# at-aaims/OmniFed

Hardware: AMD Instinct MI355X
Metric: GB/s device-resident QSGD encode+decode, Llama-400M grads, 1/2/4/8 GPUs (higher is better)
Workload: dtype f32; 1 GPU; llama400m QSGD encode+decode, bit_width 4 (16 levels, int8 wire), philox draws, client weighting fused (alpha = batch_samples = rank + 1), one client per GPU; tensors=183, elements_per_client=401122304, bit_width=4, parallelism=clients1

## Files before the change

omnifed_amd/csrc/omf_plan.h:

```cpp
#pragma once

#include <algorithm>
#include <vector>

#include "../../include/omf_codec.h"
#include "omf_common.h"
#include "omf_plan_layout.h"

namespace omf {

constexpr uint64_t kWaitTicks = 2000000ull;

struct SpecBracket {
  float c_lo, c_hi, n_lo, n_hi;
  uint32_t mode;
  uint32_t pad[3];
};

}

struct omf_plan {
  int device = 0;
  int32_t nt = 0;
  int64_t chunk = omf::plan_layout::kSub;
// ... 9 lines not shown
  void* d_block = nullptr;
  uint8_t* d_sync = nullptr;
  size_t sync_bytes = 0, off_counters = 16, off_gran = 0;
  int64_t n_enc[2] = {0, 0};
  omf::plan_layout::Item* d_enc[2] = {nullptr, nullptr};
  int64_t n_flat = 0, n_partials = 0;
  omf::plan_layout::Item* d_flat = nullptr;
  omf::plan_layout::TensorInfo* d_tinfo[2] = {nullptr, nullptr};
  uint64_t* d_partials = nullptr;
  int64_t* d_sizes = nullptr;
  int64_t* d_begins = nullptr;
  int32_t ring_cfg = 0;
  int32_t ring_grid = 0;
  int32_t ring_big_mode = 1;
  int64_t ring_gap = -1;
  int64_t ring_hold_override = 0;
  uint32_t ring_dbg = 0;
  uint32_t ring_epoch = 0;
  int64_t n_ring = 0, n_ring_gran = 0, ring_hold_max = 0, ring_two_pass = 0;
  omf::ring::Item* d_ring = nullptr;
  omf::ring::Tensor* d_ring_t = nullptr;
  uint64_t* d_ring_gran = nullptr;
  unsigned long long* d_ring_prof = nullptr;
  int64_t n_spec_blocks = 0, n_spec_fold = 0;
  omf::plan_layout::SpecBrItem* d_spec_br_items = nullptr;
  omf::plan_layout::SpecFoldItem* d_spec_fold_items = nullptr;
  uint64_t* d_spec_seg_part = nullptr;
  uint32_t* d_spec_cnt = nullptr;
  omf::SpecBracket* d_spec_br = nullptr;
  uint64_t* d_spec_ngran = nullptr;
  uint64_t* d_spec_part = nullptr;
  uint32_t* d_spec_slots = nullptr;
  uint32_t* d_spec_heads = nullptr;
  int64_t n_dec_blocks = 0;
  uint32_t* d_dec_binfo = nullptr;
  float4* d_spec_recs = nullptr;
  uint32_t* d_spec_flags = nullptr;
  uint32_t* d_spec_status = nullptr;
  int32_t grid_wgs = 0;
  uint32_t* d_grid_pbeg = nullptr;
  uint32_t* d_grid_pcnt = nullptr;
  unsigned long long* d_grid_bar = nullptr;
  uint64_t grid_launches = 0;
  uint32_t spec_epoch = 0;
  uint32_t spec_skip = 0;
  float spec_zsig = 5.0f;
  float spec_zsig_wide = 4.0f;
  int32_t spec_fb = 1;
  int32_t spec_wide = 1;
  int32_t spec_last_pw = 0;
  std::vector<void*> d_lazy;
  uint32_t* d_spec_slots_w = nullptr;
  float4* d_spec_recs_w = nullptr;
  double* d_spec_br_part = nullptr;
  uint32_t* d_spec_br_cnt = nullptr;
  double* d_spec_fb_part = nullptr;
  uint32_t* d_spec_fb_cnt = nullptr;
  uint64_t* d_spec_brgran = nullptr;
  struct TopkTable {
    uint64_t key;
    void* dev;
    uint64_t host;
    std::vector<int64_t> counts;
  };
  std::vector<TopkTable> topk_tables;
  omf::TopkKnobs topk_knobs;
// ... 69 lines not shown
```

omnifed_amd/csrc/omf_plan_layout.cpp:

```cpp
#include "omf_plan_layout.h"

#include <algorithm>
#include <utility>

namespace omf {
namespace plan_layout {

namespace {

void build_sequence(const Desc& d, bool resident_ok, std::vector<Item>& seq, std::vector<TensorInfo>& tinfo,
                    int64_t& npart) {
  seq.clear();
  tinfo.assign(d.nt, TensorInfo{});
  npart = 0;
  std::vector<Item> deferred;
  for (int32_t t = 0; t < d.nt; ++t) {
    const int64_t n = d.sizes[t], b = d.offsets[t];
    const int64_t es = (int64_t)d.ev * 1024;
    const int64_t ns = (n + es - 1) / es;
    std::vector<Item> q_t;
    if (ns == 1 || (resident_ok && ns <= d.cap)) {
      tinfo[t] = TensorInfo{b, n, es, (int32_t)ns, (int32_t)npart};
      for (int64_t c = 0; c < ns; ++c) {
        const int64_t cb = b + c * es;
// ... 151 lines not shown
    const int64_t p_begin = kItemParts * (int64_t)o.flat.size();
    for (int64_t c = 0; c * kSub < n; ++c) {
      const int64_t cb = b + c * kSub;
      o.flat.push_back(Item{cb, std::min(b + n, cb + kSub), t, kQuant, (int32_t)c, 0});
    }
    const int64_t p_end = kItemParts * (int64_t)o.flat.size();
    o.grid_pbeg[(size_t)t] = (uint32_t)(p_begin / kItemParts);
    o.grid_pcnt[(size_t)t] = (uint32_t)((p_end - p_begin) / kItemParts);
    const int64_t R = std::max<int64_t>(1, std::min<int64_t>(kSpecRuns, n / (2 * kSpecRun)));
    const int64_t Rw = std::max<int64_t>(1, std::min<int64_t>(kSpecRunsWide, n / (2 * kSpecRunWide)));
    o.br_items.push_back(SpecBrItem{b, n, n / R, (int32_t)R, (int32_t)(n % R), t, (int32_t)Rw});
    const int32_t nsegs = (int32_t)((p_end - p_begin + kSpecSeg - 1) / kSpecSeg);
    for (int32_t q = 0; q < nsegs; ++q)
      o.fold_items.push_back(SpecFoldItem{p_begin + (int64_t)q * kSpecSeg,
                                          std::min(p_end, p_begin + (int64_t)(q + 1) * kSpecSeg), t, q, nsegs, seg_base});
    seg_base += nsegs;
  }
}

void build_dec_blocks(const Desc& d, std::vector<uint32_t>& binfo) {
  const int64_t arena_end = d.offsets[d.nt - 1] + d.sizes[d.nt - 1];
  binfo.assign((size_t)((arena_end + kDecBlk - 1) / kDecBlk), 0u);
  int32_t t = 0;
  for (size_t k = 0; k < binfo.size(); ++k) {
    const int64_t base = (int64_t)k * kDecBlk;
    while (t + 1 < d.nt && d.offsets[t + 1] <= base) ++t;
    const bool inside = d.offsets[t] <= base && base + kDecBlk <= d.offsets[t] + d.sizes[t];
    binfo[k] = (uint32_t)t | (inside ? 0x80000000u : 0u);
  }
}

}

bool build_tables(const Desc& d, Tables& o) {
  int64_t np[2];
  build_sequence(d, true, o.enc[0], o.tinfo[0], np[0]);
  build_sequence(d, false, o.enc[1], o.tinfo[1], np[1]);
  build_ring_sequence(d, o);
  build_flat_tables(d, o);
  build_dec_blocks(d, o.dec_binfo);
  o.n_enc[0] = (int64_t)o.enc[0].size();
  o.n_enc[1] = (int64_t)o.enc[1].size();
  o.n_flat = (int64_t)o.flat.size();
  o.n_spec_blocks = 4 * o.n_flat;
  o.n_partials = std::max<int64_t>(std::max(np[0], np[1]), 1);
  return std::max(o.n_enc[0], o.n_spec_blocks) <= 0x7fffffffLL;
}

Choice choose_encoder(const Call& c) {
  const bool int32_wire = c.bits > 6;
  const int32_t ordered = c.strategy >= 2 ? kEncOrdered : c.strategy;
  if (c.norms_only) return {(Encoder)ordered};
  if (c.caller_norms) return {kEncCallerNorms};
  if (c.strategy == 4 && !c.caller_u && !c.divide && c.grid_fits) return {kEncGrid};
  if (c.strategy == 3 && !c.caller_u && c.bits >= kSpecMinBits) {
    const bool wide = c.bits > kSpecMaxBits;
    const bool serves = wide ? !c.last_client && c.wide_levels && c.bits <= kSpecMaxBitsWide && c.fmt == 0
                             : c.fmt == 0 || !c.divide;
    if (serves) {
      const bool skip_bracket = (c.spec_dbg & 1u) != 0;
      const bool fused = c.fused_bracket && !c.last_client && c.fmt == 0 && !skip_bracket;
      return {kEncBracket, wide, fused, !fused && !skip_bracket};
    }
  }
  const bool wide_ring = c.strategy == 3 && int32_wire && !c.caller_u && c.fmt == 0;
  if (c.strategy == 2 || c.strategy == 4 || c.divide || wide_ring) return {kEncRing};
  return {(Encoder)ordered};
}

}
}
```

omnifed_amd/csrc/omf_plan_layout.h:

```cpp
#pragma once

#include <cstddef>
#include <cstdint>
#include <vector>

namespace omf {

namespace ring {

enum : int32_t { kPublish = 1, kQuant = 2 };

struct Item {
  int64_t begin, end;
  int64_t tbegin, tn;
  int32_t tensor, flags, chunk, nchunks;
  int32_t gbase, pad[3];
};

struct Tensor {
  int64_t begin, n;
  int32_t nchunks, gbase;
  int32_t pad[2];
};

}

namespace plan_layout {

constexpr int kBlkWaves = 4;
constexpr int64_t kSub = 16384;
constexpr int64_t kSpecBlk = 4096;
constexpr int64_t kDecBlk = 4096;
constexpr int kSpecSeg = 4096;
constexpr int kSpecRun = 64;
constexpr int kSpecRuns = 512;
constexpr int kSpecRunWide = 256;
constexpr int kSpecRunsWide = 512;
#ifndef OMF_BR_PARTS
#define OMF_BR_PARTS 2
#endif
constexpr int kBrParts = OMF_BR_PARTS;
constexpr int kFbParts = 8;
#ifndef OMF_WFB_PARTS
#define OMF_WFB_PARTS 16
#endif
constexpr int kWfbParts = OMF_WFB_PARTS;
constexpr int kGridNB = 3;
constexpr int kSpecMinBits = 1;
constexpr int kSpecMaxBits = 4;
constexpr int kSpecMaxBitsWide = 8;
static_assert(kSub == 4 * kSpecBlk, "four spec blocks per flat item");

enum : int32_t { kNorm = 0, kQuant = 1, kResident = 2 };

struct Item {
  int64_t begin, end;
  int32_t tensor, kind, chunk, pad;
};

struct TensorInfo {
  int64_t begin, n;
  int64_t chunk;
  int32_t nchunks, pbase;
};

struct SpecBrItem {
  int64_t begin, n;
  int64_t base;
  int32_t R, rem;
  int32_t tensor, Rw;
};
struct SpecFoldItem {
  int64_t p_begin, p_end;
  int32_t tensor, seg, nsegs, sbase;
};

struct Desc {
  const int64_t* sizes = nullptr;
  const int64_t* offsets = nullptr;
  int32_t nt = 0;
  int64_t chunk = 2 * kSub;
  int32_t ev = 8;
  int64_t cap = 1;
  int64_t ring_chunk = kSub;
  int32_t ring_slots = 1, ring_kind = 0;
  int32_t ring_grid = 1;
  int32_t ring_big_mode = 1;
  int64_t ring_gap = -1;
  int64_t ring_hold_override = 0;
};

struct Tables {
  std::vector<Item> enc[2];
  std::vector<TensorInfo> tinfo[2];
  std::vector<Item> flat;
  std::vector<ring::Item> ring;
  std::vector<ring::Tensor> ring_t;
  std::vector<SpecBrItem> br_items;
  std::vector<SpecFoldItem> fold_items;
  std::vector<uint32_t> grid_pbeg, grid_pcnt;
  std::vector<uint32_t> dec_binfo;
  int64_t n_enc[2] = {0, 0}, n_flat = 0;
  int64_t n_partials = 0;
  int64_t n_spec_blocks = 0;
  int64_t n_ring_gran = 0;
  int64_t ring_hold_max = 0;
  int64_t ring_two_pass = 0;
};

bool build_tables(const Desc& d, Tables& out);

inline size_t round16(size_t b) { return (b + 15) & ~(size_t)15; }

class Carve {
 public:
  struct Region {
    size_t offset, bytes;
    const void* src;
    bool zero;
    void* field;
    void (*set)(void* field, void* addr);
  };
  template <class T>
  void copy(T*& field, const std::vector<T>& host) { add(field, host.size(), host.data(), false); }
  template <class T>
  void copy(T*& field, const T* host, size_t count) { add(field, count, host, false); }
  template <class T>
  void zero(T*& field, size_t count) { add(field, count, static_cast<const T*>(nullptr), true); }
  template <class T>
  void raw(T*& field, size_t count) { add(field, count, static_cast<const T*>(nullptr), false); }
  size_t bytes() const { return total_; }
  const std::vector<Region>& regions() const { return regions_; }
  void bind(void* base) const {
// ... 48 lines not shown
```

omnifed_amd/csrc/omf_qsgd.hip:

```cpp
#include <algorithm>
#include <cstdlib>
#include <cstring>
#include <type_traits>
#include <vector>

#include "../../include/omf_codec.h"
#include "../../include/omf_codec_experimental.h"
#include "omf_common.h"
#include "omf_plan.h"
#include "omf_qsgd_dev.h"
#include "omf_ring.h"

using namespace omf;
using namespace omf::plan_layout;

namespace {

constexpr int kV = 16;
static_assert(kSub == (int64_t)kV * kThreads * 4, "a flat item is one sub-chunk of a 256-thread workgroup");
static_assert(kBlkWaves == kWaves, "one wave partial per wave of a block's workgroup");

struct EncArgs {
  const float* x;
  const float* u;
// ... 796 lines not shown
        }
      }
      float acc = 0.0f;
#pragma unroll
      for (int i = 0; i < 4; ++i) acc = sq4(spec_prologue(v[i], a.e.alpha, a.divisor, a.e.fmt), acc);
      s1 += (double)acc;
    }
  } else {
    bracket_sample<kSpecRun, false, kThreads, 4>(a, x, t, tb, n, R, part, kFbParts, s1, s2);
  }
  double S1 = block_sum_f64(s1, red), S2 = block_sum_f64(s2, red);
  if (!exact) {
    if (threadIdx.x == 0) {
      double* bp = a.br_part + 2 * ((int64_t)t * kFbParts + part);
      st_agent(reinterpret_cast<uint64_t*>(bp), (uint64_t)__double_as_longlong(S1));
      st_agent(reinterpret_cast<uint64_t*>(bp + 1), (uint64_t)__double_as_longlong(S2));
      drain_vmem();
      const uint32_t last = add_agent(&a.br_cnt[t], 1u) == (uint32_t)(kFbParts - 1) ? 1u : 0u;
      if (last) __hip_atomic_store(&a.br_cnt[t], 0u, __ATOMIC_RELAXED, __HIP_MEMORY_SCOPE_AGENT);
      s_last = last;
    }
    __syncthreads();
    if (!s_last) return;
    S1 = S2 = 0.0;
    for (int g = 0; g < kFbParts; ++g) {
      const uint64_t* bp = reinterpret_cast<const uint64_t*>(a.br_part + 2 * ((int64_t)t * kFbParts + g));
      S1 += __longlong_as_double((long long)ld_agent(bp));
      S2 += __longlong_as_double((long long)ld_agent(bp + 1));
    }
  }
  if (threadIdx.x != 0) return;
  const SpecBracket o = bracket_from_sums(a, exact, n, R, kSpecRun, S1, S2);
  a.br[t] = o;
  const uint64_t ep = (uint64_t)a.epoch << 32;
  st_agent(&a.brgran[2 * t], ep | __float_as_uint(o.c_lo));
  st_agent(&a.brgran[2 * t + 1], ep | __float_as_uint(o.c_hi));
}

template <int WIDTH, bool DIV>
__global__ __launch_bounds__(kThreads) void qsgd_spec_quant_fb(SpecArgs a, const SpecBrItem* __restrict__ bitems,
                                                               int64_t nbrw, const int64_t* __restrict__ begins) {
  if ((int64_t)blockIdx.x < nbrw) {
    spec_bracket_part(a, bitems, blockIdx.x);
    return;
  }
  const int64_t blk = (int64_t)blockIdx.x - nbrw;
  const Item it = a.e.items[blk >> 2];
  const int32_t t = it.tensor;
  const int64_t tb = begins[t];
  const int64_t b = it.begin + (blk & 3) * kSpecBlk;
  const int wave = threadIdx.x >> 6;
  uint32_t* slot = a.slots + blk * kSpecSlot;
  uint64_t* part = a.partials + blk * kWaves + wave;
  if (b >= it.end) {
    if ((threadIdx.x & 63) == 0) {
      *part = 0ull;
      a.heads[blk * kWaves + wave] = (uint32_t)t << 8;
    }
    return;
  }
  auto get_br = [&]() {
    uint64_t g0 = ld_agent(&a.brgran[2 * t]), g1 = ld_agent(&a.brgran[2 * t + 1]);
    if ((uint32_t)(g0 >> 32) != a.epoch || (uint32_t)(g1 >> 32) != a.epoch) {
      const uint64_t t0 = wall_clock64(), min_polls = a.wait_ticks >> 10;
      uint64_t polls = 0;
      for (int k = 0;; k = min(k + 1, 6)) {
        if (k < 2) __builtin_amdgcn_s_sleep(2);
        else __builtin_amdgcn_s_sleep(8);
        g0 = ld_agent(&a.brgran[2 * t]);
        g1 = ld_agent(&a.brgran[2 * t + 1]);
        if ((uint32_t)(g0 >> 32) == a.epoch && (uint32_t)(g1 >> 32) == a.epoch) break;
        if (++polls > min_polls && wall_clock64() - t0 > a.wait_ticks) {
          __hip_atomic_fetch_or(&a.flags[t], 2u, __ATOMIC_RELAXED, __HIP_MEMORY_SCOPE_AGENT);
          g0 = g1 = 0;
          break;
        }
      }
    }
    SpecBracket o{__uint_as_float((uint32_t)g0), __uint_as_float((uint32_t)g1), 0.f, 0.f, 0u, {0u, 0u, 0u}};
    return o;
// ... 28 lines not shown
        v[i] = e + 4 <= n ? *reinterpret_cast<const float4*>(x + e) : make_float4(0.f, 0.f, 0.f, 0.f);
        if (e < n && e + 4 > n) {
          v[i].x = x[e];
          if (e + 1 < n) v[i].y = x[e + 1];
          if (e + 2 < n) v[i].z = x[e + 2];
        }
      }
      float acc = 0.0f;
#pragma unroll
      for (int i = 0; i < 4; ++i) acc = sq4(spec_prologue(v[i], a.e.alpha, a.divisor, a.e.fmt), acc);
      s1 += (double)acc;
    }
  } else {
    bracket_sample<kSpecRunWide, false, 64, kPassesW>(a, x, t, tb, n, R, part, kWfbParts, s1, s2);
  }
  double S1 = wave_sum_f64(s1), S2 = wave_sum_f64(s2);
  if (lane != 0) return;
  if (!exact) {
    double* bp = a.br_part + 2 * ((int64_t)t * kWfbParts + part);
    st_agent(reinterpret_cast<uint64_t*>(bp), (uint64_t)__double_as_longlong(S1));
    st_agent(reinterpret_cast<uint64_t*>(bp + 1), (uint64_t)__double_as_longlong(S2));
    drain_vmem();
    if (add_agent(&a.br_cnt[t], 1u) != (uint32_t)(kWfbParts - 1)) return;
    __hip_atomic_store(&a.br_cnt[t], 0u, __ATOMIC_RELAXED, __HIP_MEMORY_SCOPE_AGENT);
    S1 = S2 = 0.0;
    for (int g = 0; g < kWfbParts; ++g) {
      const uint64_t* q = reinterpret_cast<const uint64_t*>(a.br_part + 2 * ((int64_t)t * kWfbParts + g));
      S1 += __longlong_as_double((long long)ld_agent(q));
      S2 += __longlong_as_double((long long)ld_agent(q + 1));
    }
  }
  const SpecBracket o = bracket_from_sums(a, exact, n, R, kSpecRunWide, S1, S2);
  a.br[t] = o;
  const uint64_t ep = (uint64_t)a.epoch << 32;
  st_agent(&a.brgran[2 * t], ep | __float_as_uint(o.c_lo));
  st_agent(&a.brgran[2 * t + 1], ep | __float_as_uint(o.c_hi));
}

__device__ __forceinline__ SpecBracket fb_poll(const SpecArgs& a, int32_t t) {
  uint64_t g0 = ld_agent(&a.brgran[2 * t]), g1 = ld_agent(&a.brgran[2 * t + 1]);
  if ((uint32_t)(g0 >> 32) != a.epoch || (uint32_t)(g1 >> 32) != a.epoch) {
    const uint64_t t0 = wall_clock64(), min_polls = a.wait_ticks >> 10;
    uint64_t polls = 0;
    for (int k = 0;; k = min(k + 1, 6)) {
      if (k < 2) __builtin_amdgcn_s_sleep(2);
      else __builtin_amdgcn_s_sleep(8);
      g0 = ld_agent(&a.brgran[2 * t]);
      g1 = ld_agent(&a.brgran[2 * t + 1]);
      if ((uint32_t)(g0 >> 32) == a.epoch && (uint32_t)(g1 >> 32) == a.epoch) break;
      if (++polls > min_polls && wall_clock64() - t0 > a.wait_ticks) {
        __hip_atomic_fetch_or(&a.flags[t], 2u, __ATOMIC_RELAXED, __HIP_MEMORY_SCOPE_AGENT);
        g0 = g1 = 0;
        break;
      }
    }
  }
  return SpecBracket{__uint_as_float((uint32_t)g0), __uint_as_float((uint32_t)g1), 0.f, 0.f, 0u, {0u, 0u, 0u}};
}

template <int WIDTH, bool DIV>
__global__ __launch_bounds__(64) void qsgd_spec_quant_wfb(SpecArgs a, const SpecBrItem* __restrict__ bitems,
                                                          int64_t nbrw, const int64_t* __restrict__ begins) {
  if ((int64_t)blockIdx.x < nbrw) {
    spec_bracket_part_wide(a, bitems, blockIdx.x);
    return;
  }
  const int64_t wgi = (int64_t)blockIdx.x - nbrw;
  const int64_t blk = wgi / kWaves;
  const int tid = (int)(wgi % kWaves) * 64 + (int)threadIdx.x;
  const Item it = a.e.items[blk >> 2];
  const int32_t t = it.tensor;
  const int64_t tb = begins[t];
  const int64_t b = it.begin + (blk & 3) * kSpecBlk;
  const int wave = tid >> 6;
  uint32_t* slot = a.slots + blk * spec_slot_words(kSpecPerWaveWide);
  uint64_t* part = a.partials + blk * kWaves + wave;
  if (b >= it.end) {
    if (threadIdx.x == 0) {
      *part = 0ull;
      a.heads[blk * kWaves + wave] = (uint32_t)t << 8;
    }
    return;
  }
  auto get_br = [&]() { return fb_poll(a, t); };
  const int64_t end = min(b + kSpecBlk, it.end);
  if (end - b == kSpecBlk)
    spec_block<WIDTH, true, DIV, kFmtF32, 0, kSpecPerWaveWide>(a, blk, b, end, t, tb, get_br, slot, part, 0.0f, tid);
  else
    spec_block<WIDTH, false, DIV, kFmtF32, 0, kSpecPerWaveWide>(a, blk, b, end, t, tb, get_br, slot, part, 0.0f, tid);
}

__device__ void spec_fold(const SpecArgs& a, const SpecFoldItem& fi) {
  __shared__ double red[kWaves];
  __shared__ uint32_t s_last;
  const int32_t t = fi.tensor;
  constexpr int U = kSpecSeg / kThreads;
  double v[U];
#pragma unroll
  for (int i = 0; i < U; ++i) {
    const int64_t j = fi.p_begin + threadIdx.x + (int64_t)i * kThreads;
    const double d = __longlong_as_double((long long)a.partials[j < fi.p_end ? j : fi.p_begin]);
    v[i] = j < fi.p_end ? d : 0.0;
  }
// ... 651 lines not shown
    for (const Carve::Region& r : c.regions()) {
      void* dst = static_cast<uint8_t*>(*block) + r.offset;
      if (!r.bytes) continue;
      if (r.src) OMF_HIP(hipMemcpy(dst, r.src, r.bytes, hipMemcpyHostToDevice));
      else if (r.zero) OMF_HIP(hipMemset(dst, 0, r.bytes));
    }
    return OMF_OK;
  };
  const int rc = fill();
  if (rc != OMF_OK && *block) {
    (void)hipFree(*block);
    *block = nullptr;
  }
  c.bind(*block);
  return rc;
}

static int upload_plan(omf_plan* p) {
  const ring::Config rc = ring::config(p->ring_cfg);
  Desc d;
  d.sizes = p->sizes.data();
  d.offsets = p->offsets.data();
  d.nt = p->nt;
  d.chunk = p->chunk;
  d.ev = p->ev;
  d.cap = p->cap;
  d.ring_chunk = ring::chunk_elems(rc);
  d.ring_slots = rc.slots;
  d.ring_kind = rc.kind;
  d.ring_grid = p->ring_grid;
  d.ring_big_mode = p->ring_big_mode;
  d.ring_gap = p->ring_gap;
  d.ring_hold_override = p->ring_hold_override;
  Tables tb;
  if (!build_tables(d, tb)) return fail(OMF_EINVAL, "too many work items");
  p->n_enc[0] = tb.n_enc[0];
  p->n_enc[1] = tb.n_enc[1];
  p->n_flat = tb.n_flat;
  p->n_partials = tb.n_partials;
  p->n_ring = (int64_t)tb.ring.size();
  p->n_ring_gran = tb.n_ring_gran;
  p->ring_hold_max = tb.ring_hold_max;
  p->ring_two_pass = tb.ring_two_pass;
  p->n_spec_blocks = tb.n_spec_blocks;
  p->n_spec_fold = (int64_t)tb.fold_items.size();
  p->n_dec_blocks = (int64_t)tb.dec_binfo.size();
  p->off_counters = 16;
  p->off_gran = round16(p->off_counters + 4 * (size_t)p->nt);
  p->sync_bytes = round16(p->off_gran + 8 * (size_t)p->nt);
  const size_t nt = (size_t)p->nt, nb = (size_t)p->n_spec_blocks;
  Carve c;
  c.zero(p->d_sync, p->sync_bytes);
  c.copy(p->d_enc[0], tb.enc[0]);
  c.copy(p->d_enc[1], tb.enc[1]);
  c.copy(p->d_flat, tb.flat);
  c.copy(p->d_tinfo[0], tb.tinfo[0]);
  c.copy(p->d_tinfo[1], tb.tinfo[1]);
  c.raw(p->d_partials, (size_t)p->n_partials);
  c.copy(p->d_sizes, p->sizes);
  c.copy(p->d_begins, p->offsets);
  c.copy(p->d_ring, tb.ring);
  c.copy(p->d_ring_t, tb.ring_t);
  c.zero(p->d_ring_gran, (size_t)p->n_ring_gran);
  c.zero(p->d_ring_prof, 16);
  c.copy(p->d_spec_br_items, tb.br_items);
  c.copy(p->d_spec_fold_items, tb.fold_items);
  c.raw(p->d_spec_seg_part, tb.fold_items.size());
  c.zero(p->d_spec_cnt, nt + 1);
  c.raw(p->d_spec_br, nt);
  c.zero(p->d_spec_ngran, nt);
  c.raw(p->d_spec_part, kWaves * nb);
  c.raw(p->d_spec_slots, kSpecSlot * nb);
  c.raw(p->d_spec_heads, kWaves * nb);
  c.copy(p->d_dec_binfo, tb.dec_binfo);
  c.raw(p->d_spec_recs, 2 * (size_t)kWaves * kSpecPerWave * nb);
  c.zero(p->d_spec_flags, nt);
  c.zero(p->d_spec_status, nt);
  c.copy(p->d_grid_pbeg, tb.grid_pbeg);
  c.copy(p->d_grid_pcnt, tb.grid_pcnt);
  c.zero(p->d_grid_bar, 2);
  DeviceGuard g(p->device);
  if (!g.ok) return fail(OMF_EHIP, "hipSetDevice failed");
  if (p->d_block) {
    OMF_HIP(hipDeviceSynchronize());
    (void)hipFree(p->d_block);
    p->d_block = nullptr;
  }
  p->grid_launches = 0;
  return make_block(c, &p->d_block);
}

static int make_buffers(omf_plan* p, const Carve& c, hipStream_t st) {
  std::vector<void*> made;
  auto alloc = [&]() -> int {
    for (const Carve::Region& r : c.regions()) {
      void* d = nullptr;
      OMF_HIP(hipMalloc(&d, r.bytes));
      made.push_back(d);
      if (r.zero) OMF_HIP(hipMemsetAsync(d, 0, r.bytes, st));
    }
    return OMF_OK;
  };
  if (const int rc = alloc()) {
    for (void* d : made) (void)hipFree(d);
    c.bind(nullptr);
    return rc;
  }
  for (size_t i = 0; i < made.size(); ++i) c.regions()[i].set(c.regions()[i].field, made[i]);
  p->d_lazy.insert(p->d_lazy.end(), made.begin(), made.end());
  return OMF_OK;
}

static int ensure_wide(omf_plan* p, hipStream_t st) {
// ... 52 lines not shown
      return fail(OMF_EHIP, "omf_plan_create: cannot query the device");
    }
    if (const char* ev = omf::knob("OMF_ENCODE_ROWS")) p->ev = atoi(ev) == 16 ? 16 : 8;
    const void* k16[5] = {(const void*)qsgd_encode_ordered<1, false, false, 16>,
                          (const void*)qsgd_encode_ordered<1, true, false, 16>,
                          (const void*)qsgd_encode_ordered<4, false, false, 16>,
                          (const void*)qsgd_encode_ordered<4, true, false, 16>,
                          (const void*)qsgd_encode_ordered<1, false, true, 16>};
    const void* k8[5] = {(const void*)qsgd_encode_ordered<1, false, false, 8>,
                         (const void*)qsgd_encode_ordered<1, true, false, 8>,
                         (const void*)qsgd_encode_ordered<4, false, false, 8>,
                         (const void*)qsgd_encode_ordered<4, true, false, 8>,
                         (const void*)qsgd_encode_ordered<1, false, true, 8>};
    const void* const* kerns = p->ev == 8 ? k8 : k16;
    int nb_min = 1 << 30;
    for (int i = 0; i < 5; ++i) {
      int nb = 0;
      if (hipOccupancyMaxActiveBlocksPerMultiprocessor(&nb, kerns[i], kThreads, 0) != hipSuccess || nb < 1) nb = 1;
      nb_min = std::min(nb_min, nb);
    }
    p->cap = std::max<int64_t>(1, (int64_t)nb_min * prop.multiProcessorCount / 2);
    if (const char* rc = omf::knob("OMF_RING_CFG")) p->ring_cfg = std::max(0, std::min(atoi(rc), omf::ring::num_configs() - 1));
    if (const char* bm = omf::knob("OMF_RING_BIG")) p->ring_big_mode = atoi(bm) == 1 ? 1 : 0;
    if (const char* gp = omf::knob("OMF_RING_GAP")) p->ring_gap = atoll(gp);
#ifdef OMF_EXPERIMENTS
    if (const char* dg = omf::knob("OMF_RING_DBG")) p->ring_dbg = (uint32_t)atoi(dg);
    if (const char* sk = omf::knob("OMF_SPEC_SKIP")) p->spec_skip = (uint32_t)atoi(sk);
#endif
    if (const char* zs = omf::knob("OMF_SPEC_ZSIG")) p->spec_zsig = p->spec_zsig_wide = std::max(1.0f, (float)atof(zs));
    p->strategy = p->arena_end >= ((int64_t)1 << 25) ? 3 : 2;
    if (const char* st = omf::knob("OMF_ENCODE_STRATEGY")) p->strategy = std::max(0, std::min(atoi(st), 4));
    if (const char* sw = omf::knob("OMF_SPEC_WIDE")) p->spec_wide = atoi(sw) != 0 ? 1 : 0;
    if (const char* fb = omf::knob("OMF_SPEC_FB")) p->spec_fb = atoi(fb) != 0 ? 1 : 0;
    {
      int nb = 0;
      if (hipOccupancyMaxActiveBlocksPerMultiprocessor(&nb, (const void*)qsgd_encode_grid<1>, 1024, 0) == hipSuccess &&
          nb >= 1)
        p->grid_wgs = prop.multiProcessorCount;
    }
    p->ring_grid = omf::ring::grid_size(p->ring_cfg, device);
    if (p->ring_grid <= 0) {
      delete p;
      return fail(OMF_EHIP, "omf_plan_create: cannot size the ring encoder grid");
    }
  }
  if (int r = upload_plan(p)) {
    if (p->d_block) (void)hipFree(p->d_block);
    delete p;
    return r;
  }
  *out = p;
  return OMF_OK;
}

int omf_plan_destroy(omf_plan* plan) {
  if (!plan) return OMF_OK;
  DeviceGuard g(plan->device);
  if (plan->last_ev) (void)hipEventDestroy(plan->last_ev);
  if (plan->d_block) (void)hipFree(plan->d_block);
  for (void* d : plan->d_lazy)
    if (d) (void)hipFree(d);
  for (auto& e : plan->topk_tables) (void)hipFree(e.dev);
  delete plan;
  return OMF_OK;
}

// ... 51 lines not shown

int omf_plan_ring_profile(omf_plan* plan, int64_t* out16) {
  if (!plan || !out16) return fail(OMF_EINVAL, "omf_plan_ring_profile: NULL argument");
  DeviceGuard g(plan->device);
  OMF_HIP(hipDeviceSynchronize());
  OMF_HIP(hipMemcpy(out16, plan->d_ring_prof, 8 * 16, hipMemcpyDeviceToHost));
  OMF_HIP(hipMemset(plan->d_ring_prof, 0, 8 * 16));
  return OMF_OK;
}

int omf_plan_ring_info(const omf_plan* plan, int64_t* out) {
  if (!plan || !out) return fail(OMF_EINVAL, "omf_plan_ring_info: NULL argument");
  out[0] = plan->ring_grid;
  out[1] = omf::ring::chunk_elems(omf::ring::config(plan->ring_cfg));
  out[2] = plan->n_ring;
  out[3] = plan->ring_hold_max;
  out[4] = plan->ring_two_pass;
  out[5] = plan->ring_cfg;
  return OMF_OK;
}

int omf_plan_set_resident_capacity(omf_plan* plan, int64_t cap, int64_t wait_us) {
  if (!plan) return fail(OMF_EINVAL, "plan is NULL");
  if (cap < 0 || wait_us < 0) return fail(OMF_EINVAL, "cap and wait_us must be >= 0");
  if (cap > 0) plan->cap = cap;
  plan->wait_ticks = wait_us > 0 ? (uint64_t)wait_us * 100ull : kWaitTicks;
  if (cap > 0) return upload_plan(plan);
  return OMF_OK;
}

int omf_plan_set_debug(omf_plan* plan, uint32_t ring_dbg, uint32_t spec_dbg, int64_t lds_wait_us) {
  if (!plan) return fail(OMF_EINVAL, "plan is NULL");
  if (lds_wait_us < 0) return fail(OMF_EINVAL, "lds_wait_us must be >= 0");
  if ((ring_dbg & ~15u) || (spec_dbg & ~511u)) return fail(OMF_EINVAL, "omf_plan_set_debug: unknown switch bits");
  plan->ring_dbg = ring_dbg;
  plan->spec_skip = spec_dbg;
  plan->lds_wait_ticks = lds_wait_us > 0 ? (uint64_t)lds_wait_us * 100ull : kWaitTicks;
  return OMF_OK;
}

int omf_plan_spec_stats(omf_plan* plan, void* stream, int64_t* out4) {
  if (!plan || !out4) return fail(OMF_EINVAL, "omf_plan_spec_stats: NULL argument");
  DeviceGuard g(plan->device);
  OMF_HIP(hipStreamSynchronize((hipStream_t)stream));
  std::vector<uint32_t> status(plan->nt), heads((size_t)kWaves * (size_t)plan->n_spec_blocks);
  std::vector<SpecBracket> br(plan->nt);
  OMF_HIP(hipMemcpy(status.data(), plan->d_spec_status, 4 * (size_t)plan->nt, hipMemcpyDeviceToHost));
  OMF_HIP(hipMemcpy(br.data(), plan->d_spec_br, sizeof(SpecBracket) * (size_t)plan->nt, hipMemcpyDeviceToHost));
  OMF_HIP(hipMemcpy(heads.data(), plan->d_spec_heads, 4 * heads.size(), hipMemcpyDeviceToHost));
  int64_t whole = 0, deferred = 0, listed = 0, full = 0;
  for (int32_t t = 0; t < plan->nt; ++t) {
    whole += status[t] != 0u;
    deferred += br[t].mode != 0u;
  }
  for (int64_t blk = 0; blk < plan->n_spec_blocks; ++blk)
    for (int w = 0; w < kWaves; ++w) {
      const uint32_t c = heads[(size_t)blk * kWaves + w] & 0xffu;
      listed += c;
      full += c == (uint32_t)plan->spec_last_pw;
    }
  out4[0] = whole;
  out4[1] = deferred;
  out4[2] = listed;
  out4[3] = full;
  return OMF_OK;
}

int omf_plan_check(omf_plan* plan, void* stream) {
  if (!plan) return fail(OMF_EINVAL, "omf_plan_check: plan is NULL");
  DeviceGuard g(plan->device);
// ... 90 lines not shown
}

using EncKernel = void (*)(EncArgs);

static void launch_caller_norms(omf_plan* p, const EncCall& c) {
  static const EncKernel kern[2][2] = {
      {qsgd_quant_sub<1, false, 4, false>, qsgd_quant_sub<1, true, 4, false>},
      {qsgd_quant_sub<4, false, 4, false>, qsgd_quant_sub<4, true, 4, false>}};
  EncArgs a = enc_args(p, c);
  a.items = p->d_flat;
  a.tinfo = p->d_tinfo[0];
  launch(kern[c.width == 4][c.u != nullptr], dim3((unsigned)(p->n_flat * 4)), dim3(kThreads), 0, c.st, a);
}

static int launch_grid(omf_plan* p, const EncCall& c) {
  GridArgs ga;
  ga.e = enc_args(p, c);
  ga.e.items = p->d_flat;
  ga.partials = p->d_spec_part;
  ga.bar = p->d_grid_bar;
  ga.target = (unsigned long long)(p->grid_launches + 1) * (unsigned long long)p->grid_wgs;
  ga.nblocks = p->n_spec_blocks;
  ga.dbg = p->spec_skip;
  launch(c.width == 1 ? qsgd_encode_grid<1> : qsgd_encode_grid<4>, dim3((unsigned)p->grid_wgs), dim3(1024), 0, c.st, ga,
         p->d_flat, p->d_begins, p->d_grid_pbeg, p->d_grid_pcnt);
  OMF_HIP(hipGetLastError());
  ++p->grid_launches;
  return OMF_OK;
}

static int launch_bracket(omf_plan* p, const EncCall& c, const Choice& ch) {
  using BracketKernel = void (*)(SpecArgs, const SpecBrItem*);
  using PassKernel = void (*)(SpecArgs, const SpecBracket*, const int64_t*, const float*);
  using FusedKernel = void (*)(SpecArgs, const SpecBrItem*, int64_t, const int64_t*);
  using FinishKernel = void (*)(SpecArgs, const SpecFoldItem*, int32_t, const Item*, const int64_t*, const uint32_t*,
                                const float4*, const uint32_t*);
  constexpr int PWW = kSpecPerWaveWide;
#ifndef OMF_FIX_FT
#define OMF_FIX_FT 4
#endif
  constexpr int FT = OMF_FIX_FT;
  static const BracketKernel k_bracket[2] = {qsgd_spec_bracket<false, false>, qsgd_spec_bracket<false, true>};
  static const FusedKernel k_fb[2] = {qsgd_spec_quant_fb<1, false>, qsgd_spec_quant_fb<1, true>};
  static const FusedKernel k_wfb[2][2] = {{qsgd_spec_quant_wfb<1, false>, qsgd_spec_quant_wfb<1, true>},
                                          {qsgd_spec_quant_wfb<4, false>, qsgd_spec_quant_wfb<4, true>}};
  static const PassKernel k_pass[2][2] = {{qsgd_spec_quant<1, false>, qsgd_spec_quant<1, true>},
                                          {qsgd_spec_quant<4, false>, qsgd_spec_quant<4, true>}};
  static const PassKernel k_pass_half[2] = {qsgd_spec_quant<1, false, kFmtBF16>, qsgd_spec_quant<1, false, kFmtF16>};
  static const PassKernel k_pass_last[2] = {qsgd_spec_quant<1, true, kFmtF32, 1>,
                                            qsgd_spec_quant<1, true, kFmtF32, 4>};
  static const PassKernel k_pass_wide[2][2][2] = {
      {{qsgd_spec_quant<1, false, kFmtF32, 0, PWW, 1>, qsgd_spec_quant<1, true, kFmtF32, 0, PWW, 1>},
       {qsgd_spec_quant<4, false, kFmtF32, 0, PWW, 1>, qsgd_spec_quant<4, true, kFmtF32, 0, PWW, 1>}},
      {{qsgd_spec_quant<1, false, kFmtF32, 0, PWW>, qsgd_spec_quant<1, true, kFmtF32, 0, PWW>},
       {qsgd_spec_quant<4, false, kFmtF32, 0, PWW>, qsgd_spec_quant<4, true, kFmtF32, 0, PWW>}}};
  static const FinishKernel k_finish[2][2] = {{qsgd_spec_finish<1>, qsgd_spec_finish<4>},
                                              {qsgd_spec_finish<1, PWW, FT>, qsgd_spec_finish<4, PWW, FT>}};
  static const size_t plds_w = [] { const char* v = omf::knob("OMF_SPEC_LDS_W"); return v ? (size_t)atoi(v) : (size_t)10240; }();
  static const size_t plds_n = [] { const char* v = omf::knob("OMF_SPEC_LDS"); return v ? (size_t)atoi(v) : (size_t)24576; }();
  static const bool wpb4 = [] { const char* v = omf::knob("OMF_SPEC_WPB"); return v && atoi(v) == 4; }();

  const hipStream_t st = c.st;
  const AccIn* acc = c.acc_in;
  const bool wide = ch.wide, div = c.divisor != 0.0f, w4 = c.width == 4;
  if (wide)
    if (int r = ensure_wide(p, st)) return r;
  if (ch.fused)
// ... 12 lines not shown
  sa.epoch = p->spec_epoch;
  sa.wide = wide ? 1u : 0u;
  sa.ngran = p->d_spec_ngran;
  sa.dbg = p->spec_skip;
  sa.zsig = wide ? p->spec_zsig_wide : p->spec_zsig;
  sa.divisor = c.divisor;
  sa.xout = c.xout;
  sa.wait_ticks = p->wait_ticks;
  sa.br = p->d_spec_br;
  sa.partials = p->d_spec_part;
  sa.br_part = ch.fused ? p->d_spec_fb_part : p->d_spec_br_part;
  sa.br_cnt = ch.fused ? p->d_spec_fb_cnt : p->d_spec_br_cnt;
  sa.brgran = p->d_spec_brgran;
  p->spec_last_pw = wide ? kSpecPerWaveWide : kSpecPerWave;
  sa.slots = wide ? p->d_spec_slots_w : p->d_spec_slots;
  sa.heads = p->d_spec_heads;
  sa.recs = wide ? p->d_spec_recs_w : p->d_spec_recs;
  sa.flags = p->d_spec_flags;
  sa.status = p->d_spec_status;
  sa.nblocks = p->n_spec_blocks;
  sa.aq = acc ? acc->q : nullptr;
  sa.anorm = acc ? acc->norm : nullptr;
  sa.aout = acc ? acc->acc_out : nullptr;
  sa.awidth = acc ? acc->width : 0;
  sa.alevels = acc ? (float)acc->levels : 0.0f;
  sa.ainv = acc && (acc->levels & (acc->levels - 1)) == 0 ? 1.0f / (float)acc->levels : 0.0f;

  const int64_t nb = p->n_spec_blocks, nt = p->nt;
  if (ch.bracket_launch)
    launch(wide ? qsgd_spec_bracket_wide : k_bracket[acc != nullptr], dim3((unsigned)(nt * (wide ? kBrParts : 1))),
           dim3(kBrThreads), 0, st, sa, sa.br_items);
  if (ch.fused) {
    const int64_t nbrw = (wide ? kWfbParts : kFbParts) * nt;
    if (wide) launch(k_wfb[w4][div], dim3((unsigned)(nbrw + nb * kWaves)), dim3(64), plds_w, st, sa, sa.br_items, nbrw, sa.begins);
    else launch(k_fb[div], dim3((unsigned)(nbrw + nb)), dim3(kThreads), div ? 0 : plds_n, st, sa, sa.br_items, nbrw, sa.begins);
  } else if (wide && !wpb4) {
    launch(k_pass_wide[0][w4][div], dim3((unsigned)(nb * kWaves)), dim3(64), plds_w, st, sa, sa.br, sa.begins, sa.anorm);
  } else {
    const PassKernel k = wide                 ? k_pass_wide[1][w4][div]
                         : c.fmt == kFmtBF16 ? k_pass_half[0]
                         : c.fmt == kFmtF16  ? k_pass_half[1]
                         : acc               ? k_pass_last[acc->width == 32]
                                             : k_pass[w4][div];
    launch(k, dim3((unsigned)nb), dim3(kThreads), 0, st, sa, sa.br, sa.begins, sa.anorm);
  }
  if (!(p->spec_skip & 2u)) {
    const int64_t per = kThreads / (kWaves * (wide ? FT : 1));
    const int32_t nfold = (int32_t)p->n_spec_fold;
    launch(k_finish[wide][w4], dim3((unsigned)(nfold + (nb + per - 1) / per)), dim3(kThreads), 0, st, sa, sa.fold_items,
           nfold, sa.e.items, sa.begins, sa.slots, sa.recs, sa.heads);
  }
  OMF_HIP(hipGetLastError());
  return OMF_OK;
}

static int launch_ring(omf_plan* p, const EncCall& c) {
  omf::ring::Args r;
  r.x = c.x; r.u = c.u; r.q = c.q; r.norm_out = c.norm_out;
  r.items = p->d_ring; r.tinfo = p->d_ring_t; r.gran = p->d_ring_gran;
  r.err = p->err_word();
  r.n_items = p->n_ring;
  r.alpha = c.alpha;
  r.fmt = c.fmt;
  r.round_in = (c.fmt != 0 && c.alpha != 1.0f) ? 1u : 0u;
  r.divisor = c.divisor;
  r.divide = c.divisor != 0.0f ? 1u : 0u;
  r.xout = c.xout;
  r.levels = (float)(1u << c.s);
// ... 329 lines not shown
```

Baseline: 6430 GB/s.

## Map fused QSGD grid slots through a host-built table of bracket and block items

Replaces the fixed layout of the fused bracket+quantise kernels, where all bracket-sampling workgroups came first and block workgroups after, with a host-built per-slot GridItem table. The table can interleave each tensor's sampling workgroups near its first quantise blocks, controlled by lead and share knobs. The default lead keeps all sampling first, so the default schedule should match the old one. It adds one table load per workgroup plus new debug bits, including one that skips the bracket granule publish.

```diff
diff --git a/omnifed_amd/csrc/omf_plan.h b/omnifed_amd/csrc/omf_plan.h
--- a/omnifed_amd/csrc/omf_plan.h
+++ b/omnifed_amd/csrc/omf_plan.h
@@ -65,6 +65,11 @@
   uint64_t* d_spec_part = nullptr;
   uint32_t* d_spec_slots = nullptr;
   uint32_t* d_spec_heads = nullptr;
+  omf::plan_layout::GridItem* d_spec_gitems = nullptr;
+  omf::plan_layout::GridItem* d_spec_gitems_w = nullptr;
+  int64_t spec_lead = 0, spec_lead_wide = 0;
+  int32_t spec_share = 0, spec_share_wide = 0;
+  bool spec_lead_test = false;
   int64_t n_dec_blocks = 0;
   uint32_t* d_dec_binfo = nullptr;
   float4* d_spec_recs = nullptr;
diff --git a/omnifed_amd/csrc/omf_plan_layout.cpp b/omnifed_amd/csrc/omf_plan_layout.cpp
--- a/omnifed_amd/csrc/omf_plan_layout.cpp
+++ b/omnifed_amd/csrc/omf_plan_layout.cpp
@@ -207,6 +207,49 @@
 
 }
 
+bool build_grid_map(const int64_t* first_wg, int32_t nt, int64_t n_block_wgs, int parts, int64_t lead, int share,
+                    std::vector<uint32_t>& map) {
+  map.clear();
+  if (nt <= 0 || parts <= 0 || kMapStride % parts != 0 || share < parts || share > kMapStride) return false;
+  const int64_t total = (int64_t)nt * parts + n_block_wgs;
+  if ((int64_t)nt * parts >= ((int64_t)1 << 24) || total > 0x7fffffffLL) return false;
+  const int64_t reach = lead < 0 ? -1 : std::min<int64_t>(lead, total) + kMapStride;
+  int32_t ts = 0;
+  int64_t be = 0;
+  for (int64_t g = 0; g < total; g += kMapStride) {
+    const int64_t before = (int64_t)ts * parts;
+    int64_t nin = 0;
+    while (ts < nt && nin + parts <= kMapStride && (ts == 0 || reach < 0 || first_wg[ts] - be < reach) &&
+           (nin + parts <= share || first_wg[ts] - be < kMapStride)) {
+      ++ts;
+      nin += parts;
+    }
+    map.push_back((uint32_t)(before << 8) | (uint32_t)nin);
+    be += kMapStride - nin;
+  }
+  return ts == nt;
+}
+
+bool build_grid_items(const std::vector<uint32_t>& map, int64_t total, int per, const std::vector<Item>& flat,
+                      std::vector<GridItem>& out) {
+  out.clear();
+  if (per <= 0 || kMapStride % per != 0 || total % per != 0) return false;
+  for (int64_t idx = 0; idx < total; idx += per) {
+    int64_t first, last;
+    const uint32_t entry = map[(size_t)(idx >> kMapShift)];
+    const bool sample = grid_map_slot(entry, (uint32_t)idx, first);
+    if (grid_map_slot(entry, (uint32_t)(idx + per - 1), last) != sample || last != first + per - 1) return false;
+    if (sample) {
+      out.push_back(GridItem{0, 0, -1, (int32_t)first, 0, 1});
+    } else {
+      if (first % per != 0 || first / per >= (int64_t)flat.size()) return false;
+      const Item& it = flat[(size_t)(first / per)];
+      out.push_back(GridItem{it.begin, it.end, it.tensor, (int32_t)(first / per), it.chunk, 0});
+    }
+  }
+  return true;
+}
+
 bool build_tables(const Desc& d, Tables& o) {
   int64_t np[2];
   build_sequence(d, true, o.enc[0], o.tinfo[0], np[0]);
@@ -219,7 +262,17 @@
   o.n_flat = (int64_t)o.flat.size();
   o.n_spec_blocks = 4 * o.n_flat;
   o.n_partials = std::max<int64_t>(std::max(np[0], np[1]), 1);
-  return std::max(o.n_enc[0], o.n_spec_blocks) <= 0x7fffffffLL;
+  if (std::max(o.n_enc[0], o.n_spec_blocks) > 0x7fffffffLL) return false;
+  std::vector<int64_t> first((size_t)d.nt);
+  for (int32_t t = 0; t < d.nt; ++t) first[(size_t)t] = (kSub / kSpecBlk) * (int64_t)o.grid_pbeg[(size_t)t];
+  if (!build_grid_map(first.data(), d.nt, o.n_spec_blocks, kFbParts, d.spec_lead, d.spec_share, o.gmap)) return false;
+  for (int64_t& f : first) f *= kBlkWaves;
+  if (!build_grid_map(first.data(), d.nt, o.n_spec_blocks * kBlkWaves, kWfbParts, d.spec_lead_wide, d.spec_share_wide,
+                      o.gmap_wide))
+    return false;
+  return build_grid_items(o.gmap, (int64_t)d.nt * kFbParts + o.n_spec_blocks, kGridPer, o.flat, o.gitems) &&
+         build_grid_items(o.gmap_wide, (int64_t)d.nt * kWfbParts + o.n_spec_blocks * kBlkWaves, kGridPerWide, o.flat,
+                          o.gitems_wide);
 }
 
 Choice choose_encoder(const Call& c) {
diff --git a/omnifed_amd/csrc/omf_plan_layout.h b/omnifed_amd/csrc/omf_plan_layout.h
--- a/omnifed_amd/csrc/omf_plan_layout.h
+++ b/omnifed_amd/csrc/omf_plan_layout.h
@@ -51,12 +51,55 @@
 constexpr int kSpecMaxBitsWide = 8;
 static_assert(kSub == 4 * kSpecBlk, "four spec blocks per flat item");
 
+constexpr int kMapShift = 6;
+constexpr int64_t kMapStride = (int64_t)1 << kMapShift;
+constexpr int64_t kLeadAllFirst = -1;
+constexpr int64_t kLeadTwoGen = 2 * 256 * 6, kLeadTwoGenWide = 2 * 256 * 16;
+constexpr int kGridPer = (int)(kSub / kSpecBlk);
+constexpr int kGridPerWide = kGridPer * kBlkWaves;
+static_assert(kMapStride % kFbParts == 0 && kMapStride % kWfbParts == 0,
+              "a chunk takes whole tensors' sampling workgroups: it is full or has room for one more");
+static_assert(kFbParts % kGridPer == 0 && kWfbParts % kGridPerWide == 0 && kMapStride % kGridPerWide == 0,
+              "a group of slots is all sampling workgroups or one flat item's blocks");
+static_assert(kMapStride <= 0xff, "the count of a chunk's sampling workgroups is a byte");
+
+#if defined(__HIPCC__)
+#define OMF_LAYOUT_HD __host__ __device__
+#else
+#define OMF_LAYOUT_HD
+#endif
+OMF_LAYOUT_HD inline bool grid_map_slot(uint32_t entry, uint32_t idx, int64_t& index) {
+  const uint32_t r = idx & (uint32_t)(kMapStride - 1), nin = entry & 0xffu, before = entry >> 8;
+  if (r < nin) {
+    index = (int64_t)(before + r);
+    return true;
+  }
+  index = (int64_t)idx - (int64_t)(before + nin);
+  return false;
+}
+
+struct GridItem {
+  int64_t begin, end;
+  int32_t tensor, index, chunk, sample;
+};
+OMF_LAYOUT_HD inline bool grid_item_slot(const GridItem& g, uint32_t idx, int per, int64_t& index) {
+  const uint32_t r = idx % (uint32_t)per;
+  index = g.sample ? (int64_t)g.index + r : (int64_t)g.index * per + r;
+  return g.sample != 0;
+}
+
+bool build_grid_map(const int64_t* first_wg, int32_t nt, int64_t n_block_wgs, int parts, int64_t lead, int share,
+                    std::vector<uint32_t>& map);
+
 enum : int32_t { kNorm = 0, kQuant = 1, kResident = 2 };
 
 struct Item {
   int64_t begin, end;
   int32_t tensor, kind, chunk, pad;
 };
+
+bool build_grid_items(const std::vector<uint32_t>& map, int64_t total, int per, const std::vector<Item>& flat,
+                      std::vector<GridItem>& out);
 
 struct TensorInfo {
   int64_t begin, n;
@@ -88,6 +131,9 @@
   int32_t ring_big_mode = 1;
   int64_t ring_gap = -1;
   int64_t ring_hold_override = 0;
+  int64_t spec_lead = kLeadAllFirst;
+  int64_t spec_lead_wide = kLeadAllFirst;
+  int32_t spec_share = (int32_t)kMapStride, spec_share_wide = (int32_t)kMapStride;
 };
 
 struct Tables {
@@ -99,6 +145,8 @@
   std::vector<SpecBrItem> br_items;
   std::vector<SpecFoldItem> fold_items;
   std::vector<uint32_t> grid_pbeg, grid_pcnt;
+  std::vector<uint32_t> gmap, gmap_wide;
+  std::vector<GridItem> gitems, gitems_wide;
   std::vector<uint32_t> dec_binfo;
   int64_t n_enc[2] = {0, 0}, n_flat = 0;
   int64_t n_partials = 0;
diff --git a/omnifed_amd/csrc/omf_qsgd.hip b/omnifed_amd/csrc/omf_qsgd.hip
--- a/omnifed_amd/csrc/omf_qsgd.hip
+++ b/omnifed_amd/csrc/omf_qsgd.hip
@@ -852,6 +852,7 @@
   if (threadIdx.x != 0) return;
   const SpecBracket o = bracket_from_sums(a, exact, n, R, kSpecRun, S1, S2);
   a.br[t] = o;
+  if (a.dbg & 512u) return;
   const uint64_t ep = (uint64_t)a.epoch << 32;
   st_agent(&a.brgran[2 * t], ep | __float_as_uint(o.c_lo));
   st_agent(&a.brgran[2 * t + 1], ep | __float_as_uint(o.c_hi));
@@ -859,13 +860,14 @@
 
 template <int WIDTH, bool DIV>
 __global__ __launch_bounds__(kThreads) void qsgd_spec_quant_fb(SpecArgs a, const SpecBrItem* __restrict__ bitems,
-                                                               int64_t nbrw, const int64_t* __restrict__ begins) {
-  if ((int64_t)blockIdx.x < nbrw) {
-    spec_bracket_part(a, bitems, blockIdx.x);
+                                                               const GridItem* __restrict__ gitems,
+                                                               const int64_t* __restrict__ begins) {
+  const GridItem it = gitems[blockIdx.x / kGridPer];
+  int64_t blk;
+  if (grid_item_slot(it, blockIdx.x, kGridPer, blk)) {
+    spec_bracket_part(a, bitems, blk);
     return;
   }
-  const int64_t blk = (int64_t)blockIdx.x - nbrw;
-  const Item it = a.e.items[blk >> 2];
   const int32_t t = it.tensor;
   const int64_t tb = begins[t];
   const int64_t b = it.begin + (blk & 3) * kSpecBlk;
@@ -960,6 +962,7 @@
   }
   const SpecBracket o = bracket_from_sums(a, exact, n, R, kSpecRunWide, S1, S2);
   a.br[t] = o;
+  if (a.dbg & 512u) return;
   const uint64_t ep = (uint64_t)a.epoch << 32;
   st_agent(&a.brgran[2 * t], ep | __float_as_uint(o.c_lo));
   st_agent(&a.brgran[2 * t + 1], ep | __float_as_uint(o.c_hi));
@@ -988,15 +991,16 @@
 
 template <int WIDTH, bool DIV>
 __global__ __launch_bounds__(64) void qsgd_spec_quant_wfb(SpecArgs a, const SpecBrItem* __restrict__ bitems,
-                                                          int64_t nbrw, const int64_t* __restrict__ begins) {
-  if ((int64_t)blockIdx.x < nbrw) {
-    spec_bracket_part_wide(a, bitems, blockIdx.x);
+                                                          const GridItem* __restrict__ gitems,
+                                                          const int64_t* __restrict__ begins) {
+  const GridItem it = gitems[blockIdx.x / kGridPerWide];
+  int64_t wgi;
+  if (grid_item_slot(it, blockIdx.x, kGridPerWide, wgi)) {
+    spec_bracket_part_wide(a, bitems, wgi);
     return;
   }
-  const int64_t wgi = (int64_t)blockIdx.x - nbrw;
   const int64_t blk = wgi / kWaves;
   const int tid = (int)(wgi % kWaves) * 64 + (int)threadIdx.x;
-  const Item it = a.e.items[blk >> 2];
   const int32_t t = it.tensor;
   const int64_t tb = begins[t];
   const int64_t b = it.begin + (blk & 3) * kSpecBlk;
@@ -1714,6 +1718,10 @@
   d.ring_big_mode = p->ring_big_mode;
   d.ring_gap = p->ring_gap;
   d.ring_hold_override = p->ring_hold_override;
+  d.spec_lead = p->spec_lead_test ? kLeadTwoGen : p->spec_lead;
+  d.spec_lead_wide = p->spec_lead_test ? kLeadTwoGenWide : p->spec_lead_wide;
+  d.spec_share = p->spec_share;
+  d.spec_share_wide = p->spec_share_wide;
   Tables tb;
   if (!build_tables(d, tb)) return fail(OMF_EINVAL, "too many work items");
   p->n_enc[0] = tb.n_enc[0];
@@ -1761,6 +1769,8 @@
   c.copy(p->d_grid_pbeg, tb.grid_pbeg);
   c.copy(p->d_grid_pcnt, tb.grid_pcnt);
   c.zero(p->d_grid_bar, 2);
+  c.copy(p->d_spec_gitems, tb.gitems);
+  c.copy(p->d_spec_gitems_w, tb.gitems_wide);
   DeviceGuard g(p->device);
   if (!g.ok) return fail(OMF_EHIP, "hipSetDevice failed");
   if (p->d_block) {
@@ -1879,6 +1889,14 @@
     if (const char* st = omf::knob("OMF_ENCODE_STRATEGY")) p->strategy = std::max(0, std::min(atoi(st), 4));
     if (const char* sw = omf::knob("OMF_SPEC_WIDE")) p->spec_wide = atoi(sw) != 0 ? 1 : 0;
     if (const char* fb = omf::knob("OMF_SPEC_FB")) p->spec_fb = atoi(fb) != 0 ? 1 : 0;
+    p->spec_lead = Desc().spec_lead;
+    p->spec_lead_wide = Desc().spec_lead_wide;
+    if (const char* ld = omf::knob("OMF_SPEC_LEAD")) p->spec_lead = std::max<int64_t>(atoll(ld), kLeadAllFirst);
+    if (const char* ld = omf::knob("OMF_SPEC_LEAD_W")) p->spec_lead_wide = std::max<int64_t>(atoll(ld), kLeadAllFirst);
+    p->spec_share = Desc().spec_share;
+    p->spec_share_wide = Desc().spec_share_wide;
+    if (const char* sh = omf::knob("OMF_SPEC_SHARE")) p->spec_share = std::max(kFbParts, std::min(atoi(sh), (int)kMapStride));
+    if (const char* sh = omf::knob("OMF_SPEC_SHARE_W")) p->spec_share_wide = std::max(kWfbParts, std::min(atoi(sh), (int)kMapStride));
     {
       int nb = 0;
       if (hipOccupancyMaxActiveBlocksPerMultiprocessor(&nb, (const void*)qsgd_encode_grid<1>, 1024, 0) == hipSuccess &&
@@ -1996,10 +2014,15 @@
 int omf_plan_set_debug(omf_plan* plan, uint32_t ring_dbg, uint32_t spec_dbg, int64_t lds_wait_us) {
   if (!plan) return fail(OMF_EINVAL, "plan is NULL");
   if (lds_wait_us < 0) return fail(OMF_EINVAL, "lds_wait_us must be >= 0");
-  if ((ring_dbg & ~15u) || (spec_dbg & ~511u)) return fail(OMF_EINVAL, "omf_plan_set_debug: unknown switch bits");
+  if ((ring_dbg & ~15u) || (spec_dbg & ~2047u)) return fail(OMF_EINVAL, "omf_plan_set_debug: unknown switch bits");
   plan->ring_dbg = ring_dbg;
   plan->spec_skip = spec_dbg;
   plan->lds_wait_ticks = lds_wait_us > 0 ? (uint64_t)lds_wait_us * 100ull : kWaitTicks;
+  const bool lead_test = (spec_dbg & 1024u) != 0;
+  if (lead_test != plan->spec_lead_test) {
+    plan->spec_lead_test = lead_test;
+    return upload_plan(plan);
+  }
   return OMF_OK;
 }
 
@@ -2156,7 +2179,7 @@
 static int launch_bracket(omf_plan* p, const EncCall& c, const Choice& ch) {
   using BracketKernel = void (*)(SpecArgs, const SpecBrItem*);
   using PassKernel = void (*)(SpecArgs, const SpecBracket*, const int64_t*, const float*);
-  using FusedKernel = void (*)(SpecArgs, const SpecBrItem*, int64_t, const int64_t*);
+  using FusedKernel = void (*)(SpecArgs, const SpecBrItem*, const GridItem*, const int64_t*);
   using FinishKernel = void (*)(SpecArgs, const SpecFoldItem*, int32_t, const Item*, const int64_t*, const uint32_t*,
                                 const float4*, const uint32_t*);
   constexpr int PWW = kSpecPerWaveWide;
@@ -2235,8 +2258,8 @@
            dim3(kBrThreads), 0, st, sa, sa.br_items);
   if (ch.fused) {
     const int64_t nbrw = (wide ? kWfbParts : kFbParts) * nt;
-    if (wide) launch(k_wfb[w4][div], dim3((unsigned)(nbrw + nb * kWaves)), dim3(64), plds_w, st, sa, sa.br_items, nbrw, sa.begins);
-    else launch(k_fb[div], dim3((unsigned)(nbrw + nb)), dim3(kThreads), div ? 0 : plds_n, st, sa, sa.br_items, nbrw, sa.begins);
+    if (wide) launch(k_wfb[w4][div], dim3((unsigned)(nbrw + nb * kWaves)), dim3(64), plds_w, st, sa, sa.br_items, p->d_spec_gitems_w, sa.begins);
+    else launch(k_fb[div], dim3((unsigned)(nbrw + nb)), dim3(kThreads), div ? 0 : plds_n, st, sa, sa.br_items, p->d_spec_gitems, sa.begins);
   } else if (wide && !wpb4) {
     launch(k_pass_wide[0][w4][div], dim3((unsigned)(nb * kWaves)), dim3(64), plds_w, st, sa, sa.br, sa.begins, sa.anorm);
   } else {
```

Result: no change. 6421 GB/s (-0.1%).
